# rl-tools/raptor

Measured on AMD Instinct MI355X. Metric: env-steps/sec (whole node) at 65536 quadrotors per GPU, higher is better.
Workload: dtype f32; 1 GPU; 65536 parallel quadrotors per GPU, fp32 RK4 dynamics + fp32 GRU actor (RAPTOR checkpoint), domain-randomised params, auto-reset, fused rollout; envs_per_gpu=65536, total_envs=65536, episode_length=500, parallelism=single GPU, mode=fused, engine=hip, device=AMD Radeon Graphics, exchange=none (one rank: nothing to gather)

## Files before the change

### include/raptor_quad.h

```cpp
#ifndef RAPTOR_QUAD_H
#define RAPTOR_QUAD_H

#include <stddef.h>
#include <stdint.h>

#ifdef __cplusplus
extern "C" {
#endif

#define RQ_ABI_VERSION 5

#if defined(__GNUC__)
#define RQ_API __attribute__((visibility("default")))
#else
#define RQ_API
#endif

#define RQ_POLICY_INPUT_DIM 22
#define RQ_POLICY_HIDDEN_DIM 16
#define RQ_POLICY_OUTPUT_DIM 4
#define RQ_POLICY_NUM_WEIGHTS 2084
#define RQ_ACTION_DIM 4
#define RQ_OBSERVATION_DIM 26

// ... 378 lines not shown
RQ_API int rq_allgather_returns(rq_env* env, rq_comm* comm);
RQ_API int rq_comm_gathered(rq_comm* comm, const float** dev_ptr, uint32_t* count, float* host_out);

RQ_API int rq_device_timer_start(rq_device* dev);
RQ_API int rq_device_timer_stop(rq_device* dev, float* elapsed_ms);
RQ_API int rq_device_set_rollout_timing(rq_device* dev, int enable);
RQ_API int rq_device_last_rollout_ms(rq_device* dev, float* kernel_ms);
RQ_API int rq_device_last_rollout_waves(rq_device* dev, uint64_t* records, uint32_t capacity, uint32_t* n_waves);
RQ_API int rq_device_last_rollout_clock(rq_device* dev, float* core_ghz);
RQ_API int rq_device_launch_floor(rq_device* dev, uint32_t n, uint32_t reps, float* us_per_launch);
RQ_API int rq_device_set_speculation(rq_device* dev, int enable);
RQ_API int rq_device_set_resident(rq_device* dev, int enable);
RQ_API int rq_device_get_resident(const rq_device* dev, int* enabled, int* running, uint64_t* starts, uint64_t* commands, uint64_t* replays);
RQ_API int rq_device_get_resident_timing(const rq_device* dev, uint64_t* ticks6);
RQ_API int rq_device_get_speculation(const rq_device* dev, int* enabled, int* suspended, uint32_t* consecutive_misses);

#ifdef __cplusplus
}
#endif
#endif
```

### raptor_amd/_lib.py

```python
import ctypes as C
import os

_PKG = os.path.dirname(os.path.abspath(__file__))
LIB_PATH = os.environ.get("RAPTOR_QUAD_LIB") or os.path.join(_PKG, "libraptor_quad.so")

POLICY_INPUT_DIM = 22
POLICY_HIDDEN_DIM = 16
POLICY_OUTPUT_DIM = 4
POLICY_NUM_WEIGHTS = 2084
ACTION_DIM = 4
OBSERVATION_DIM = 26
PARAM_DIM = 26
STATE_DIM = 27

ROLLOUT_FUSED, ROLLOUT_CHAINED = 0, 1
ROLLOUT_AUTORESET = 1
POLICY_FP32, POLICY_BF16_MFMA, POLICY_F16X2_MFMA = 0, 1, 2
ACT_IDENTITY, ACT_RELU, ACT_TANH = 0, 1, 2
COMM_ID_BYTES = 128


class RaptorQuadError(RuntimeError):
    def __init__(self, status, message):
        super().__init__(f"libraptor_quad status {status}: {message}")
# ... 51 lines not shown
    "rq_last_error": [],
    "rq_status_string": [C.c_int],
    "rq_device_count": [C.POINTER(C.c_int)],
    "rq_device_create": [C.c_int, C.POINTER(_vp)],
    "rq_device_destroy": [_vp],
    "rq_device_synchronize": [_vp],
    "rq_device_timer_start": [_vp],
    "rq_device_timer_stop": [_vp, _fp],
    "rq_device_launch_floor": [_vp, C.c_uint32, C.c_uint32, _fp],
    "rq_device_set_rollout_timing": [_vp, C.c_int],
    "rq_device_last_rollout_ms": [_vp, _fp],
    "rq_device_last_rollout_waves": [_vp, C.c_void_p, C.c_uint32, _u32p],
    "rq_device_last_rollout_clock": [_vp, _fp],
    "rq_device_set_speculation": [_vp, C.c_int],
    "rq_device_get_speculation": [_vp, C.POINTER(C.c_int), C.POINTER(C.c_int), _u32p],
    "rq_device_set_resident": [_vp, C.c_int],
    "rq_device_get_resident_timing": [_vp, C.POINTER(C.c_uint64)],
    "rq_device_get_resident": [_vp, C.POINTER(C.c_int), C.POINTER(C.c_int), C.POINTER(C.c_uint64), C.POINTER(C.c_uint64), C.POINTER(C.c_uint64)],
    "rq_device_stream": [_vp, C.POINTER(_vp)],
    "rq_rng_create": [_vp, C.POINTER(_vp)],
    "rq_rng_destroy": [_vp],
    "rq_initialize_rng": [_vp, _vp, C.c_uint64],
    "rq_rng_get": [_vp, C.POINTER(C.c_uint64), _u32p],
    "rq_rng_set_epoch": [_vp, C.c_uint32],
    "rq_env_create": [_vp, C.c_uint32, C.c_uint64, C.POINTER(_vp)],
    "rq_env_destroy": [_vp],
    "rq_env_num_envs": [_vp, _u32p],
    "rq_env_leading_dim": [_vp, _u32p],
    "rq_env_default_config": [C.POINTER(EnvConfig)],
    "rq_initialize_environment": [_vp, _vp],
# ... 292 lines not shown
```

### raptor_amd/csrc/rq_capi.cpp

```cpp
#include "rq_objects.hpp"

namespace rq {

thread_local std::string g_last_error;
thread_local int tl_scope_depth = 0, tl_scope_device = -1;

int fail(int status, const std::string& msg) {
    try { g_last_error = msg; } catch (...) { g_last_error.clear(); }
    return status;
}

}

namespace rqh {

bool device_registry(const void* dev, int op) {
    static std::mutex m;
    static std::unordered_set<const void*> live;
    std::lock_guard<std::mutex> lock(m);
    if (op > 0) { live.insert(dev); return true; }
    if (op < 0) { live.erase(dev); return false; }
    return live.count(dev) != 0;
}

// ... 167 lines not shown
    DeviceScope on_device(ordinal);
    if (on_device.rc) return on_device.rc;
    rq_device* d = new (std::nothrow) rq_device();
    RQ_REQUIRE(d, RQ_ERR_OUT_OF_MEMORY, "host allocation failed");
    d->ordinal = ordinal;
    hipError_t e1 = hipStreamCreateWithFlags(&d->stream, hipStreamNonBlocking);
    hipError_t e2 = hipEventCreate(&d->ev_start);
    hipError_t e3 = hipEventCreate(&d->ev_stop);
    if (e3 == hipSuccess) e3 = hipEventCreateWithFlags(&d->ev_h2d, hipEventDisableTiming);
    if (e1 != hipSuccess || e2 != hipSuccess || e3 != hipSuccess) {
        delete d;
        return fail(RQ_ERR_HIP, "rq_device_create: stream/event creation failed");
    }
    d->graphs_enabled = std::getenv("RQ_NO_GRAPHS") == nullptr;
    small_batch_setup(d);
    resident_setup(d);
    device_registry(d, +1);
    *out = d;
    return RQ_OK;
}

RQ_API int rq_device_destroy(rq_device* dev) {
    if (!dev) return RQ_OK;
    DeviceScope on_device(dev->ordinal);
    resident_teardown(dev);
    device_registry(dev, -1);
    if (dev->stream) { (void)hipStreamSynchronize(dev->stream); (void)hipStreamDestroy(dev->stream); }
    if (dev->ev_start) (void)hipEventDestroy(dev->ev_start);
    if (dev->ev_stop) (void)hipEventDestroy(dev->ev_stop);
    if (dev->ev_h2d) (void)hipEventDestroy(dev->ev_h2d);
// ... 106 lines not shown
    DeviceScope on_device(dev); int rc = on_device.rc; if (rc) return rc;
    RQ_HIP(dev->rows.reserve(dev->stream, n));
    for (int i = 0; i < 3; ++i) RQ_HIP(rq::launch_fill_f32(dev->stream, dev->rows, 0.0f, n));
    RQ_HIP(hipEventRecord(dev->ev_start, dev->stream));
    for (uint32_t i = 0; i < reps; ++i) RQ_HIP(rq::launch_fill_f32(dev->stream, dev->rows, 0.0f, n));
    RQ_HIP(hipEventRecord(dev->ev_stop, dev->stream));
    RQ_HIP(hipEventSynchronize(dev->ev_stop));
    float ms = 0.0f;
    RQ_HIP(hipEventElapsedTime(&ms, dev->ev_start, dev->ev_stop));
    *us_per_launch = ms * 1e3f / (float)reps;
    return RQ_OK;
}

RQ_API int rq_device_stream(rq_device* dev, void** hip_stream) {
    RQ_REQUIRE(dev && hip_stream, RQ_ERR_INVALID_ARGUMENT, "null argument");
    *hip_stream = (void*)dev->stream;
    return RQ_OK;
}

RQ_API int rq_rng_create(rq_device* dev, rq_rng** out) {
    RQ_REQUIRE(dev && out, RQ_ERR_INVALID_ARGUMENT, "null argument");
    rq_rng* r = new (std::nothrow) rq_rng();
    RQ_REQUIRE(r, RQ_ERR_OUT_OF_MEMORY, "host allocation failed");
    r->dev = dev;
    *out = r;
    return RQ_OK;
}

RQ_API int rq_rng_destroy(rq_rng* rng) { delete rng; return RQ_OK; }

// ... 148 lines not shown
    delete p;
    return RQ_OK;
}
RQ_API int rq_params_get(const rq_params* p, float* host_out) {
    RQ_REQUIRE(p && host_out, RQ_ERR_INVALID_ARGUMENT, "null argument");
    return soa_to_host(p->env->dev, p->d, p->env->n, p->env->ld, RQ_PARAM_DIM, host_out);
}
RQ_API int rq_params_set(rq_params* p, const float* host_in) {
    RQ_REQUIRE(p && host_in, RQ_ERR_INVALID_ARGUMENT, "null argument");
    p->version = fresh_version();
    return host_to_soa(p->env->dev, host_in, p->env->n, RQ_PARAM_DIM, p->env->ld, RQ_PARAM_DIM, p->d);
}
RQ_API int rq_params_device_ptr(const rq_params* p, float** dev_ptr) {
    RQ_REQUIRE(p && dev_ptr, RQ_ERR_INVALID_ARGUMENT, "null argument");
    const_cast<rq_params*>(p)->exposed = true;
    *dev_ptr = p->d; return RQ_OK;
}

RQ_API int rq_state_create(rq_env* env, rq_state** out) {
    RQ_REQUIRE(env && out, RQ_ERR_INVALID_ARGUMENT, "null argument");
    DeviceScope on_device(env->dev); int rc = on_device.rc; if (rc) return rc;
    rq_state* s = new (std::nothrow) rq_state();
    RQ_REQUIRE(s, RQ_ERR_OUT_OF_MEMORY, "host allocation failed");
    s->env = env; s->ordinal = env->ordinal;
    const size_t bytes = (size_t)RQ_STATE_DIM * env->ld * sizeof(float);
    hipError_t e = hipMalloc(&s->d, bytes);
    s->refs = new (std::nothrow) int(1);
    if (e != hipSuccess || !s->refs) {
        if (e == hipSuccess) (void)hipFree(s->d);
        delete s->refs; delete s;
// ... 86 lines not shown
```

### raptor_amd/csrc/rq_capi_rollout.cpp

```cpp
#include "rq_objects.hpp"

#include <cmath>

namespace rqh {

int traj_block_to_host(rq_device* dev, const float* d_soa, uint32_t steps, uint32_t n, uint32_t ld, uint32_t dim,
                              float* host) {
    const size_t per_step = (size_t)n * dim * sizeof(float);
    uint32_t chunk = (uint32_t)std::min<size_t>(steps, std::max<size_t>(1, ((size_t)1 << 30) / per_step));
    if (chunk > 65535u) chunk = 65535u;
    RQ_HIP(dev->rows.reserve(dev->stream, (size_t)n * dim * chunk));
    for (uint32_t s0 = 0; s0 < steps; s0 += chunk) {
        const uint32_t c = std::min(chunk, steps - s0);
        RQ_HIP(rq::launch_soa_to_rows(dev->stream, d_soa + (size_t)s0 * dim * ld, ld, dim, n, dev->rows, c));
        RQ_HIP(hipMemcpyAsync(host + (size_t)s0 * n * dim, dev->rows, per_step * c, hipMemcpyDeviceToHost, dev->stream));
        RQ_HIP(hipStreamSynchronize(dev->stream));
    }
    return RQ_OK;
}

int rollout_check(RolloutFrame& f, const RolloutCall& c, bool actor) {
    const rq_trajectory* traj = c.traj;
    int rc = check_env_objects(c.dev, c.env, c.params, c.state); if (rc) return rc;
    RQ_REFUSE(c.who, c.params && c.state && actor && c.rng, RQ_ERR_INVALID_ARGUMENT, "null argument");
// ... 119 lines not shown
    rq_device* dev = c.dev;
    if (dev->k_timing && c.n_steps) {
        const uint32_t waves = (c.env->n + 63u) / 64u;
        const hipError_t e = dev->k_span.reserve(dev->stream, (size_t)waves * 5);
        if (e != hipSuccess) return hip_failed(c.who, "dev->k_span.reserve(dev->stream, (size_t)waves * 5)", e);
        dev->k_span_used = waves;
    }
    a.span = dev->k_timing ? dev->k_span.get() : nullptr;
    const hipError_t e = rq::launch_rollout_fused(dev->stream, a);
    if (e != hipSuccess) return hip_failed(c.who, "rq::launch_rollout_fused", e);
    dev->k_timed = dev->k_timing && c.n_steps > 0;
    dev->k_fetched = false;
    return RQ_OK;
}

}

using namespace rqh;

namespace {

struct PolicyActor {
    static constexpr bool kFoldAndReplay = true;
    rq_policy* policy;
    bool given() const { return policy != nullptr; }
    int check(const RolloutCall& c, const RolloutFrame& f) const {
        RQ_REFUSE(c.who, policy->dev == c.dev, RQ_ERR_SHAPE_MISMATCH, "policy lives on another device");
        RQ_REFUSE(c.who, !c.tables || policy->sas_mode == RQ_SAS_OFF, RQ_ERR_INVALID_ARGUMENT,
                  "tracked rollouts do not carry the SampleAndSquash stage");
        for (int k = 0; k < kScheduleKinds && c.mode == RQ_ROLLOUT_FUSED; ++k) {
            if (!f.sched[k].rows) continue;
            if (policy->precision != RQ_POLICY_FP32) return refuses_fused(c.who, k, "a bf16 / f16x2 policy");
            if (policy->sas_mode != RQ_SAS_OFF) return refuses_fused(c.who, k, "a policy with a SampleAndSquash stage");
        }
        return RQ_OK;
    }
    int prepare(const RolloutCall& c) const {
        const int rc = policy_size(policy, c.env->n); if (rc) return rc;
        RQ_REFUSE(c.who, policy->ld == c.env->ld, RQ_ERR_SHAPE_MISMATCH, "policy batch does not match the env");
        return RQ_OK;
    }
    int fused(const RolloutCall& c, const RolloutFrame& f) const {
        rq::FusedArgs a = fused_args(c, f);
        a.hidden = policy->hidden; a.weights = policy->w_dev;
        a.precision = policy->precision; a.images = packed_of(policy); a.interval = policy->native_interval;
        a.sas = sas_of(policy, c.rng->epoch, nullptr, c.env->offset);
        return fused_launch(c, a);
    }
    rq::EnvStepLaunch env_step(const RolloutCall& c, const RolloutFrame& f) const {
        rq::EnvStepLaunch e = env_step_launch(c, f);
        e.hidden = policy->hidden; e.weights = policy->w_dev;
        return e;
    }
    hipError_t thaw(const RolloutCall& c, const RolloutFrame& f) const { return rq::launch_thaw_frozen(c.dev->stream, env_step(c, f)); }
    hipError_t act(const RolloutCall& c, const RolloutFrame&, uint32_t epoch, const uint32_t* epoch_base) const {
        const rq_env* env = c.env;
        rq::ActorStepLaunch a;
        a.n = env->n; a.packed = packed_of(policy); a.precision = policy->precision;
        a.obs = env->obs; a.ld_obs = env->ld; a.hidden = policy->hidden; a.ld_h = policy->ld; a.act = env->act; a.ld_act = env->ld;
        a.frozen = env->st.frozen;
        a.sas = sas_of(policy, epoch, epoch_base, env->offset);
// ... 94 lines not shown
}

template <typename T>
int env_schedule_get(const char* who, int kind, const rq_env* env, T** bank, uint32_t* id_out) {
    RQ_REFUSE(who, env && bank, RQ_ERR_INVALID_ARGUMENT, "null argument");
    const auto& slot = env->schedule[kind];
    *bank = static_cast<T*>(slot.bank);
    if (slot.bank && id_out) std::memcpy(id_out, slot.ids.data(), (size_t)env->n * sizeof(uint32_t));
    return RQ_OK;
}

}

extern "C" {

RQ_API int rq_rollout(rq_device* dev, rq_env* env, const rq_params* params, rq_state* state, rq_policy* policy,
               rq_rng* rng, uint32_t n_steps, int mode, uint32_t flags) {
    return rollout_run({__func__, dev, env, params, state, rng, n_steps, mode, flags, nullptr, nullptr, nullptr}, PolicyActor{policy});
}

RQ_API int rq_rollout_record(rq_device* dev, rq_env* env, const rq_params* params, rq_state* state, rq_policy* policy,
                      rq_rng* rng, uint32_t n_steps, int mode, uint32_t flags, rq_trajectory* trajectory) {
    RQ_REQUIRE(trajectory, RQ_ERR_INVALID_ARGUMENT, "null trajectory");
    return rollout_run({__func__, dev, env, params, state, rng, n_steps, mode, flags, trajectory, nullptr, nullptr}, PolicyActor{policy});
}

RQ_API int rq_rollout_track(rq_device* dev, rq_env* env, const rq_params* params, rq_state* state, rq_policy* policy,
                     rq_rng* rng, uint32_t n_steps, int mode, uint32_t flags, rq_trajectory* trajectory,
                     const rq_reference* reference) {
    RQ_REQUIRE(reference, RQ_ERR_INVALID_ARGUMENT, "null reference");
// ... 164 lines not shown
```

### raptor_amd/csrc/rq_host.hpp

```cpp
#pragma once
#include <hip/hip_runtime_api.h>

#include <cstdint>
#include <string>

#include "../../include/raptor_quad.h"

namespace rq {

int fail(int status, const std::string& msg);

extern thread_local int tl_scope_depth, tl_scope_device;

struct DeviceScope {
    int previous = -1, target, rc = RQ_OK;
    bool nested = false;
    explicit DeviceScope(int ordinal) : target(ordinal) {
        if (tl_scope_depth > 0 && tl_scope_device == target) { nested = true; ++tl_scope_depth; return; }
        if (hipGetDevice(&previous) != hipSuccess) previous = -1;
        if (previous != target) {
            const hipError_t e = hipSetDevice(target);
            if (e != hipSuccess) rc = fail(RQ_ERR_HIP, std::string("hipSetDevice -> ") + hipGetErrorString(e));
        }
        outer_depth = tl_scope_depth; outer_device = tl_scope_device;
        tl_scope_depth = 1; tl_scope_device = target;
    }
    explicit DeviceScope(const rq_device* dev);
    DeviceScope(const rq_device* dev, struct KeepResident);
    ~DeviceScope() {
        if (nested) { --tl_scope_depth; return; }
        tl_scope_depth = outer_depth; tl_scope_device = outer_device;
        if (previous >= 0 && previous != target) (void)hipSetDevice(previous);
    }
// ... 34 lines not shown
```

### raptor_amd/csrc/rq_kernels.hpp

```cpp
#pragma once
#include <hip/hip_runtime_api.h>
#include <stdint.h>
#include "../../include/raptor_quad.h"
#include "rq_fused_route.hpp"
#include "rq_loss_launch.hpp"
#include "rq_step_launch.hpp"

namespace rq {

inline StepCfg step_cfg(const rq_env_config& c) {
    return {c.dt, c.gravity, c.episode_step_limit, c.reward_scale, c.reward_constant,
            c.reward_termination_penalty, c.reward_position, c.reward_orientation,
            c.reward_linear_velocity, c.reward_angular_velocity, c.reward_action,
            c.termination_enabled, c.termination_position, c.termination_linear_velocity,
            c.termination_angular_velocity, c.action_history_raw};
}
inline NoiseCfg noise_cfg(const rq_env_config& c) {
    return {c.noise_position, c.noise_orientation, c.noise_linear_velocity, c.noise_angular_velocity};
}
inline bool noise_enabled(const rq_env_config& c) {
    return c.noise_position > 0.f || c.noise_orientation > 0.f || c.noise_linear_velocity > 0.f ||
           c.noise_angular_velocity > 0.f;
}
inline SampleCfg sample_cfg(const rq_env_config& c) {
// ... 5 lines not shown
}

struct TrajPtrs {
    float* obs; float* act; float* rew; uint8_t* done;
    uint32_t t0;
};

struct TrackPtrs {
    const float* ref;
    uint32_t rows;
    uint32_t row0_at;
    float* sq;
    uint32_t* steps;
};
static_assert(sizeof(TrackPtrs) == 32, "the kernels' argument blocks hold TrackPtrs by value");

struct ResidentArgs {
    Batch b; StepCfg c; SampleCfg sc; uint64_t seed;
    const float* params; float* act; StatsPtrs st;
    float* obs_buf[2];
    const float* packed;
    float* hidden[2];
    uint32_t ld_h; float* pol_act;
    const float* rows_action;
    const uint32_t* small_rows;
    float* rows_obs;
    float* rows_act;
    uint32_t* flag;
    volatile uint32_t* packet;
    uint32_t* exited;
// ... 153 lines not shown
    bool noise = false, autoreset = false;
    const float* params = nullptr; float* state = nullptr; float* hidden = nullptr;
    const float* weights = nullptr;
    StatsPtrs st{};
    TrajPtrs traj{};
    TrackPtrs trk{};
    WrenchPtrs wr{};
    VehiclePtrs vh{};
    WindPtrs wd{};
    int precision = RQ_POLICY_FP32;
    const float* images = nullptr; const uint32_t* block_policy = nullptr; const uint32_t* policy_interval = nullptr;
    SasArgs sas{};
    uint32_t interval = 1;
    bool bank_rated = false;
    unsigned long long* span = nullptr;
};
inline FusedTraits fused_traits(const FusedArgs& a) {
    return {a.b.n, a.precision, a.sas.mode != RQ_SAS_OFF, a.trk.ref != nullptr, a.wr.rows != nullptr, a.interval,
            a.block_policy != nullptr, a.bank_rated, a.vh.rows != nullptr, a.wd.rows != nullptr};
}
hipError_t launch_rollout_fused(hipStream_t s, const FusedArgs& a);
hipError_t launch_soa_to_rows(hipStream_t s, const float* soa, uint32_t ld, uint32_t dim, uint32_t n, float* rows,
                              uint32_t slabs = 1);
hipError_t launch_rows_to_soa(hipStream_t s, const float* rows, uint32_t stride, uint32_t dim, uint32_t n, uint32_t ld,
                              float* soa);

hipError_t launch_fill_f32(hipStream_t s, float* p, float v, uint32_t count);

}
```

### raptor_amd/csrc/rq_objects.hpp

```cpp
#pragma once
#include <hip/hip_runtime_api.h>

#include <algorithm>
#include <atomic>
#include <cstdint>
#include <cstdio>
#include <cstdlib>
#include <cstring>
#include <ctime>
#include <emmintrin.h>
#include <mutex>
#include <new>
#include <string>
#include <unordered_set>
#include <utility>
#include <vector>

#include "../../include/raptor_quad.h"
#include "rq_kernels.hpp"

#include "rq_host.hpp"
#include "rq_memory.hpp"
#include "rq_call_memory.hpp"
#include "rq_env_schedule.hpp"
// ... 68 lines not shown
    const rq_params* params = nullptr; uint64_t params_version = 0;
    const rq_state* state[2] = {nullptr, nullptr};
    uint64_t version[2] = {0, 0};
    uint32_t seq = 0, n = 0;
    bool in_alt = false;
};
struct Speculation {
    bool enabled = true;
    rq_policy* last_policy = nullptr;
    rq_policy* policy = nullptr; uint64_t policy_version = 0;
    uint32_t batch = 0, seq = 0, oc_seq = 0;
    bool outstanding = false;
    bool suspended = false; uint32_t misses = 0;
};
constexpr uint32_t kSpeculationMissLimit = 4;

struct rq_device {
    int ordinal = 0;
    hipStream_t stream = nullptr;
    hipEvent_t ev_start = nullptr, ev_stop = nullptr;
    DeviceBuffer<unsigned long long> k_span;
    uint32_t k_span_used = 0;
    std::vector<unsigned long long> k_host;
    bool k_fetched = false;
    double k_ticks_per_ms = 1e5;
    bool graphs_enabled = true;
    uint32_t graph_fallbacks = 0;
    bool k_timing = false;
    bool k_timed = false;
    PinnedBuffer<float> staging;
    DeviceBuffer<float> rows;
    DeviceBuffer<float> rows2;
    PinnedBuffer<float> staging_in;
    hipEvent_t ev_h2d = nullptr;
    bool h2d_pending = false;
    HostMailbox mailbox;
    ObservationCache obs_cache;
    Speculation spec;
    ResidentExecutor resident;
};
struct rq_rng {
    rq_device* dev = nullptr;
    uint64_t seed = 0;
    uint32_t epoch = 0;
    uint32_t param_epoch = 0;
    bool initialized = false;
};

namespace rqh {
struct RowTables {
    const rq_device* dev = nullptr;
    int ordinal = 0;
    uint32_t n_tables = 0, rows = 0;
// ... 292 lines not shown
int require_bank_native_rate(const rq_policy_bank* bank, const char* what);

struct RolloutCall {
    const char* who;
    rq_device* dev; rq_env* env; const rq_params* params; rq_state* state; rq_rng* rng;
    uint32_t n_steps; int mode; uint32_t flags; rq_trajectory* traj;
    const RowTables* tables;
    const uint32_t* reference_id;
};
struct RolloutFrame {
    rq::TrajPtrs tp{nullptr, nullptr, nullptr, nullptr, 0};
    rq::TrackPtrs trk{};
    uint64_t row0_gen = 0;
    SchedulePtrs sched[kScheduleKinds];
    rq::Batch b; rq::StepCfg sc; rq::NoiseCfg nc; rq::SampleCfg smp; bool noise;
};
#define RQ_REFUSE(who, cond, status, msg)                                          \
    do {                                                                           \
        if (!(cond)) return rq::fail((status), std::string(who) + ": " + (msg));   \
    } while (0)
int rollout_check(RolloutFrame& f, const RolloutCall& c, bool actor);
int rollout_check_tables(const RolloutCall& c);
int rollout_track(RolloutFrame& f, const RolloutCall& c);
int rollout_begin(RolloutFrame& f, const RolloutCall& c);
void rollout_end(const RolloutCall& c);
int first_rows_failed(const char* what, const rq::FirstRowsStatus& s);
inline int hip_failed(const char* who, const char* what, hipError_t e) {
    return fail(e == hipErrorOutOfMemory ? RQ_ERR_OUT_OF_MEMORY : RQ_ERR_HIP, std::string(who) + ": " + what + " -> " + hipGetErrorString(e));
}
#define RQ_HIP_AS(who, expr)                                                \
    do {                                                                    \
        const hipError_t e_ = (expr);                                       \
        if (e_ != hipSuccess) return rqh::hip_failed((who), #expr, e_);     \
    } while (0)
rq::FusedArgs fused_args(const RolloutCall& c, const RolloutFrame& f);
int fused_launch(const RolloutCall& c, rq::FusedArgs& a);
rq::EnvStepLaunch env_step_launch(const RolloutCall& c, const RolloutFrame& f);

constexpr uint32_t kGraphSteps = 25;
constexpr size_t kMaxGraphs = 8;

template <typename Actor>
int rollout_chained(const RolloutCall& c, const RolloutFrame& f, const Actor& actor) {
    rq_device* dev = c.dev; rq_env* env = c.env; const rq_rng* rng = c.rng;
    const uint32_t n_steps = c.n_steps;
    const bool fold = Actor::kFoldAndReplay && !c.traj;
    const char* what = "";
    auto one_step = [&](uint32_t epoch, const uint32_t* epoch_base, uint32_t t_record) -> hipError_t {
        hipError_t e = hipSuccess;
        if (!fold) {
            what = "rq::launch_observe";
// ... 61 lines not shown
                    RQ_HIP(hipGraphLaunch(exec, dev->stream));
            }
        }
    }
    for (uint32_t t = done_steps; t < n_steps; ++t)
        if ((e = one_step(rng->epoch + t, nullptr, t)) != hipSuccess) return hip_failed(c.who, what, e);
    return RQ_OK;
}

template <typename Actor>
int rollout_run(const RolloutCall& c, Actor actor) {
    RolloutFrame f;
    int rc = rollout_check(f, c, actor.given()); if (rc) return rc;
    rc = actor.check(c, f); if (rc) return rc;
    rc = rollout_check_tables(c); if (rc) return rc;
    DeviceScope on_device(c.dev); rc = on_device.rc; if (rc) return rc;
    rc = actor.prepare(c); if (rc) return rc;
    rc = rollout_track(f, c); if (rc) return rc;
    rc = rollout_begin(f, c); if (rc) return rc;
    rc = c.mode == RQ_ROLLOUT_FUSED ? actor.fused(c, f) : rollout_chained(c, f, actor); if (rc) return rc;
    rollout_end(c);
    return RQ_OK;
}
int traj_block_to_host(rq_device* dev, const float* d_soa, uint32_t steps, uint32_t n, uint32_t ld, uint32_t dim, float* host);

template <typename T>
int copy_out(const rq_env* env, const T* src, T* dst, int dst_is_device) {
    RQ_REQUIRE(env && dst, RQ_ERR_INVALID_ARGUMENT, "null argument");
    DeviceScope on_device(env->dev); int rc = on_device.rc; if (rc) return rc;
    RQ_REQUIRE(CallMemory::valid(dst_is_device), RQ_ERR_INVALID_ARGUMENT, "dst_is_device must be 0, 1 or 2");
    CallMemory mem(dst_is_device, env->dev->stream, env->dev->ordinal);
    RQ_HIP(hipMemcpyAsync(dst, src, (size_t)env->n * sizeof(T),
                          dst_is_device ? hipMemcpyDeviceToDevice : hipMemcpyDeviceToHost, env->dev->stream));
    RQ_HIP(mem.finish());
    return RQ_OK;
}
// ... 14 lines not shown
```

### raptor_amd/csrc/rq_rollout.hpp

```cpp
#pragma once
#include <hip/hip_ext.h>

#include <cstdlib>
#include <type_traits>

#include "rq_device_math.hpp"
#include "rq_dispatch.hpp"

namespace rq {

static constexpr int kBlock = 256;
static constexpr int kFusedBlock = 64;

template <bool NT, class T>
__device__ __forceinline__ void put(T* p, T v) {
    if constexpr (NT) __builtin_nontemporal_store(v, p);
    else *p = v;
}
static constexpr bool kNtObs = true, kNtTraj = true;
static constexpr int kNtTrajAux = 2;

__device__ __forceinline__ uint32_t env_index() { return blockIdx.x * blockDim.x + threadIdx.x; }

template <typename T>
__device__ __forceinline__ T* field(T* base, uint32_t f, uint32_t ld) { return base + (size_t)f * ld; }

template <typename A> struct WavesPerSimd { static constexpr int value = 1; static constexpr bool bf16 = false; };
template <> struct WavesPerSimd<ActorF32Lean> { static constexpr int value = 2; static constexpr bool bf16 = false; };
template <> struct WavesPerSimd<ActorBF16> { static constexpr int value = 1; static constexpr bool bf16 = true; };
template <> struct WavesPerSimd<ActorF16X2> { static constexpr int value = 1; static constexpr bool bf16 = true; };


template <bool NOISE, bool AUTORESET, bool RECORD, bool SAS, typename ACTOR>
__global__ __launch_bounds__(kFusedBlock, WavesPerSimd<ACTOR>::value) void k_rollout_fused(Batch b, StepCfg c, NoiseCfg nc, SampleCfg sc,
                                                               uint64_t seed, uint32_t epoch0, uint32_t n_steps,
                                                               const float* __restrict__ params,
                                                               float* __restrict__ state,
                                                               float* __restrict__ hidden,
                                                               const float* __restrict__ w,
                                                               const float* __restrict__ packed, StatsPtrs st,
                                                               TrajPtrs traj, SasArgs sas,
                                                               unsigned long long* __restrict__ span) {
    constexpr bool TRACK = false, RATE = false, WRENCH = false;
    constexpr TrackPtrs trk{};
    constexpr WrenchPtrs wr{};
    constexpr bool VEHICLE = false;
    constexpr VehiclePtrs vh{};
    constexpr bool WIND = false;
    constexpr WindPtrs wd{};
    constexpr uint32_t interval = 1;
#include "rq_rollout_body.inc"
}

template <bool NOISE, bool AUTORESET, bool RECORD, typename ACTOR>
__global__ __launch_bounds__(kFusedBlock, WavesPerSimd<ACTOR>::value) void k_rollout_fused_track(Batch b, StepCfg c, NoiseCfg nc, SampleCfg sc,
                                                               uint64_t seed, uint32_t epoch0, uint32_t n_steps,
                                                               const float* __restrict__ params,
                                                               float* __restrict__ state,
                                                               float* __restrict__ hidden,
                                                               const float* __restrict__ w,
                                                               const float* __restrict__ packed, StatsPtrs st,
                                                               TrajPtrs traj, TrackPtrs trk,
                                                               unsigned long long* __restrict__ span) {
    constexpr bool TRACK = true, SAS = false, RATE = false, WRENCH = false;
    constexpr SasArgs sas{};
    constexpr WrenchPtrs wr{};
// ... 21 lines not shown
    constexpr bool VEHICLE = false;
    constexpr VehiclePtrs vh{};
    constexpr bool WIND = false;
    constexpr WindPtrs wd{};
#include "rq_rollout_body.inc"
}

hipError_t launch_rollout_fused_16bit(hipStream_t s, const FusedArgs& a, FusedFamily family);

inline unsigned fused_grid(const FusedArgs& a) { return (a.b.n + kFusedBlock - 1) / kFusedBlock; }

template <bool SAS, typename ACTOR>
inline void launch_fused_actor(hipStream_t s, const FusedArgs& a) {
    dispatch_bools([&](auto NZ, auto AR, auto RC) {
        hipLaunchKernelGGL((k_rollout_fused<NZ(), AR(), RC(), SAS, ACTOR>), dim3(fused_grid(a)), dim3(kFusedBlock), 0, s,
                           a.b, a.c, a.nc, a.sc, a.seed, a.epoch0, a.n_steps, a.params, a.state, a.hidden, a.weights, a.images,
                           a.st, a.traj, a.sas, a.span);
    }, a.noise, a.autoreset, a.traj.obs != nullptr);
}

template <typename ACTOR>
inline void launch_fused_track_actor(hipStream_t s, const FusedArgs& a) {
    dispatch_bools([&](auto NZ, auto AR, auto RC) {
        hipLaunchKernelGGL((k_rollout_fused_track<NZ(), AR(), RC(), ACTOR>), dim3(fused_grid(a)), dim3(kFusedBlock), 0, s,
                           a.b, a.c, a.nc, a.sc, a.seed, a.epoch0, a.n_steps, a.params, a.state, a.hidden, a.weights, a.images,
                           a.st, a.traj, a.trk, a.span);
    }, a.noise, a.autoreset, a.traj.obs != nullptr);
}

template <typename ACTOR>
inline void launch_fused_rate_actor(hipStream_t s, const FusedArgs& a) {
// ... 9 lines not shown
```

### raptor_amd/csrc/rq_rollout_body.inc

```
    unsigned long long t_in = 0;
    if (span != nullptr) t_in = (unsigned long long)wall_clock64();
    const uint32_t i0 = env_index();
    const uint32_t wave_base = i0 & ~63u;
    const uint32_t i = i0 < b.n ? i0 : b.n - 1;
    const bool valid = i0 < b.n;
    const size_t ld = b.ld;
    const uint64_t genv = b.env_offset + i;
    uint32_t ep = AUTORESET ? st.episode[i] : 0u;
    float hover_rpm = 0.0f;
    if (AUTORESET) hover_rpm = field(params, RQ_P_HOVER_RPM, ld)[i];
    const EnvConsts k = make_consts([&](int f) { return field(params, f, ld)[i]; });
    QuadState y;
    f32x2 LA01, LA23;
    float f6[6], hQ[4][4];
    y.load([&](int j) { return field(state, j, ld)[i]; });
    LA01 = f32x2{field(state, (RQ_S_LAST_ACTION + 0), ld)[i], field(state, (RQ_S_LAST_ACTION + 1), ld)[i]};
    LA23 = f32x2{field(state, (RQ_S_LAST_ACTION + 2), ld)[i], field(state, (RQ_S_LAST_ACTION + 3), ld)[i]};
#pragma unroll
    for (int j = 0; j < 6; ++j) f6[j] = field(state, (RQ_S_FORCE + j), ld)[i];
    load_hidden_q(hidden, ld, wave_base, b.n, hQ);
    float ep_ret = st.returns[i];
    uint32_t ep_steps = st.steps[i];
    float last_r = st.last_reward[i];
    float trk_sq = 0.0f;
// ... 259 lines not shown
                    if ((ended_mask & ~pre_mask) != 0) refill();
                }
                if (ended) {
                    take_presampled();
                    ds = make_disturbance(k, c.gravity, f6);
                }
                pre_mask &= ~ended_mask;
                select_hidden_q(ended_mask, h0Q, hQ);
                actor.reset_carry(ended_mask, hQ, carry);
            }
        }
    }
    };
    unsigned long long t_loop = 0, t_done = 0, c_loop = 0, c_done = 0;
    if (span != nullptr) { t_loop = (unsigned long long)wall_clock64(); c_loop = (unsigned long long)__builtin_readcyclecounter(); }
    if (sym_tau) rollout_loop(std::true_type{});
    else         rollout_loop(std::false_type{});
    if (span != nullptr) { c_done = (unsigned long long)__builtin_readcyclecounter(); t_done = (unsigned long long)wall_clock64(); }

    const bool commit = AUTORESET || !was_frozen;
    if (!AUTORESET && n_steps > 0 && last_step + 1 != n_steps) last_d = 4;
    if (AUTORESET) last_d = last_t ? 1 : (ep_steps == 0 ? 2 : 0);
    uint32_t ie = i;
    asm volatile("" : "+v"(ie));
    size_t lde = ld;
    asm volatile("" : "+s"(lde));
    if (valid && commit) {
        y.store([&](int j, float v) { field(state, j, lde)[ie] = v; });
        field(state, (RQ_S_LAST_ACTION + 0), lde)[ie] = LA01[0]; field(state, (RQ_S_LAST_ACTION + 1), lde)[ie] = LA01[1];
        field(state, (RQ_S_LAST_ACTION + 2), lde)[ie] = LA23[0]; field(state, (RQ_S_LAST_ACTION + 3), lde)[ie] = LA23[1];
        st.returns[ie] = ep_ret;
        st.steps[ie] = ep_steps;
// ... 25 lines not shown
```

### raptor_amd/l2f.py

```python
import ctypes as C
import json
import weakref

import numpy as np

from . import _lib, schedules
from ._lib import (ACTION_DIM, OBSERVATION_DIM, PARAM_DIM, STATE_DIM, ROLLOUT_AUTORESET, ROLLOUT_CHAINED,
                   ROLLOUT_FUSED, EnvConfig, RaptorQuadError)

__all__ = ["Device", "Reference", "WrenchBank", "VehicleBank", "WindBank", "UI", "vector", "vector8", "EnvConfig", "RaptorQuadError"]


class UI:

    def __init__(self, ns=""):
        self.ns = ns


class Device:

    def __init__(self, ordinal=0):
        h = C.c_void_p()
        _lib.call("rq_device_create", int(ordinal), C.byref(h))
        self._h = h
# ... 33 lines not shown
        _lib.call("rq_device_last_rollout_clock", self._h, C.byref(ghz))
        return float(ghz.value)

    def launch_floor(self, n, reps=200):
        us = C.c_float()
        _lib.call("rq_device_launch_floor", self._h, int(n), int(reps), C.byref(us))
        return float(us.value)

    def set_speculation(self, enable):
        _lib.call("rq_device_set_speculation", self._h, 1 if enable else 0)

    def speculation(self):
        e, s, m = C.c_int(), C.c_int(), C.c_uint32()
        _lib.call("rq_device_get_speculation", self._h, C.byref(e), C.byref(s), C.byref(m))
        return {"enabled": bool(e.value), "suspended": bool(s.value), "consecutive_misses": int(m.value)}

    def set_resident(self, enable):
        _lib.call("rq_device_set_resident", self._h, 1 if enable else 0)

    def resident(self):
        e, r = C.c_int(), C.c_int()
        a, b, c = C.c_uint64(), C.c_uint64(), C.c_uint64()
        _lib.call("rq_device_get_resident", self._h, C.byref(e), C.byref(r), C.byref(a), C.byref(b), C.byref(c))
        return {"enabled": bool(e.value), "running": bool(r.value), "starts": int(a.value), "commands": int(b.value), "replays": int(c.value)}

    def resident_timing_us(self):
        t = (C.c_uint64 * 6)()
        _lib.call("rq_device_get_resident_timing", self._h, t)
        return {k: (int(t[i + 1]) - int(t[0])) / 100.0 for i, k in enumerate(("rows_read", "stepped", "first_flag", "acted", "done"))}

# ... 696 lines not shown
```

Baseline: 22.96 billion env-steps/s.

## Let a running fused rollout kernel absorb steps from later rollout calls

```diff
diff --git a/include/raptor_quad.h b/include/raptor_quad.h
--- a/include/raptor_quad.h
+++ b/include/raptor_quad.h
@@ -416,6 +416,8 @@
 RQ_API int rq_device_get_resident(const rq_device* dev, int* enabled, int* running, uint64_t* starts, uint64_t* commands, uint64_t* replays);
 RQ_API int rq_device_get_resident_timing(const rq_device* dev, uint64_t* ticks6);
 RQ_API int rq_device_get_speculation(const rq_device* dev, int* enabled, int* suspended, uint32_t* consecutive_misses);
+RQ_API int rq_device_set_rollout_extension(rq_device* dev, int enable);
+RQ_API int rq_device_get_rollout_extension(rq_device* dev, int* enabled, uint64_t* launches, uint64_t* absorbed, uint64_t* continued);
 
 #ifdef __cplusplus
 }
diff --git a/raptor_amd/_lib.py b/raptor_amd/_lib.py
--- a/raptor_amd/_lib.py
+++ b/raptor_amd/_lib.py
@@ -89,6 +89,8 @@
     "rq_device_last_rollout_clock": [_vp, _fp],
     "rq_device_set_speculation": [_vp, C.c_int],
     "rq_device_get_speculation": [_vp, C.POINTER(C.c_int), C.POINTER(C.c_int), _u32p],
+    "rq_device_set_rollout_extension": [_vp, C.c_int],
+    "rq_device_get_rollout_extension": [_vp, C.POINTER(C.c_int), C.POINTER(C.c_uint64), C.POINTER(C.c_uint64), C.POINTER(C.c_uint64)],
     "rq_device_set_resident": [_vp, C.c_int],
     "rq_device_get_resident_timing": [_vp, C.POINTER(C.c_uint64)],
     "rq_device_get_resident": [_vp, C.POINTER(C.c_int), C.POINTER(C.c_int), C.POINTER(C.c_uint64), C.POINTER(C.c_uint64), C.POINTER(C.c_uint64)],
diff --git a/raptor_amd/csrc/rq_capi.cpp b/raptor_amd/csrc/rq_capi.cpp
--- a/raptor_amd/csrc/rq_capi.cpp
+++ b/raptor_amd/csrc/rq_capi.cpp
@@ -4,6 +4,7 @@
 
 thread_local std::string g_last_error;
 thread_local int tl_scope_depth = 0, tl_scope_device = -1;
+std::atomic<uint64_t> g_scopes_entered[kScopeCounters];
 
 int fail(int status, const std::string& msg) {
     try { g_last_error = msg; } catch (...) { g_last_error.clear(); }
@@ -205,6 +206,7 @@
     }
     d->graphs_enabled = std::getenv("RQ_NO_GRAPHS") == nullptr;
     small_batch_setup(d);
+    d->extend.enabled = std::getenv("RQ_NO_ROLLOUT_EXTENSION") == nullptr;
     resident_setup(d);
     device_registry(d, +1);
     *out = d;
@@ -341,6 +343,7 @@
 
 RQ_API int rq_device_stream(rq_device* dev, void** hip_stream) {
     RQ_REQUIRE(dev && hip_stream, RQ_ERR_INVALID_ARGUMENT, "null argument");
+    rq::scope_entered(dev->ordinal);
     *hip_stream = (void*)dev->stream;
     return RQ_OK;
 }
@@ -519,6 +522,7 @@
 RQ_API int rq_params_device_ptr(const rq_params* p, float** dev_ptr) {
     RQ_REQUIRE(p && dev_ptr, RQ_ERR_INVALID_ARGUMENT, "null argument");
     const_cast<rq_params*>(p)->exposed = true;
+    rq::scope_entered(p->ordinal);
     *dev_ptr = p->d; return RQ_OK;
 }
 
diff --git a/raptor_amd/csrc/rq_capi_rollout.cpp b/raptor_amd/csrc/rq_capi_rollout.cpp
--- a/raptor_amd/csrc/rq_capi_rollout.cpp
+++ b/raptor_amd/csrc/rq_capi_rollout.cpp
@@ -157,6 +157,54 @@
     return RQ_OK;
 }
 
+int extend_plan(const RolloutCall& c, const RolloutFrame& f, const rq_policy* pol, uint64_t version_in, bool ready_in, rq::FusedArgs& a) {
+    rq_device* dev = c.dev;
+    RolloutExtension& x = dev->extend;
+    const bool was_open = x.open;
+    x.open = false; x.pending = false;
+    if (!x.enabled || dev->k_timing || !rq::fused_extends(a) || c.params->exposed || c.state->exposed || c.n_steps >= rq::kExtendMaxTotal)
+        return RQ_OK;
+    if (x.agree.empty()) {
+        RQ_HIP_AS(c.who, x.agree.alloc(2));
+        RQ_HIP_AS(c.who, hipMemsetAsync(x.agree, 0, 2 * sizeof(unsigned long long), dev->stream));
+    }
+    if (x.request.empty()) {
+        RQ_HIP_AS(c.who, x.request.alloc(1));
+        *x.request.get() = 0;
+    }
+    const bool continues = was_open && ready_in && x.scopes == f.scopes_in && x.env == c.env && x.env_uid == c.env->uid &&
+                           std::memcmp(&x.cfg, &c.env->cfg, sizeof(rq_env_config)) == 0 && x.params == c.params &&
+                           x.params_version == c.params->version && x.params_d == a.params && x.state == c.state &&
+                           x.state_version == c.state->version && x.state_d == a.state && x.policy == pol &&
+                           x.policy_version == version_in && x.weight_version == pol->weight_version && x.hidden == a.hidden &&
+                           x.image == a.images && x.rng == c.rng && x.seed == a.seed && x.next_epoch == a.epoch0 &&
+                           x.total + c.n_steps <= rq::kExtendMaxTotal;
+    x.seq = (x.seq + 1) & 0x7FFFFFFFu;
+    if (x.seq == 0) x.seq = 1;
+    if (continues) { a.ext.start = x.total; x.total += c.n_steps; ++x.continued; }
+    else           { a.ext.start = 0; x.total = c.n_steps; ++x.window; }
+    __atomic_store_n(x.request.get(), ((unsigned long long)x.window << 32) | x.total, __ATOMIC_RELEASE);
+    a.ext.agree = x.agree; a.ext.request = x.request; a.ext.counts = reinterpret_cast<uint32_t*>(x.agree.get() + 1);
+    a.ext.seq = x.seq; a.ext.window = x.window; a.ext.epoch0 = a.epoch0;
+    x.env = c.env; x.env_uid = c.env->uid; x.cfg = c.env->cfg;
+    x.params = c.params; x.params_version = c.params->version; x.params_d = a.params;
+    x.state = c.state; x.state_d = a.state;
+    x.policy = pol; x.policy_version = pol->version; x.weight_version = pol->weight_version; x.hidden = a.hidden; x.image = a.images;
+    x.rng = c.rng; x.seed = a.seed;
+    x.pending = true;
+    return RQ_OK;
+}
+
+void extend_launched(const RolloutCall& c) {
+    RolloutExtension& x = c.dev->extend;
+    if (!x.pending) return;
+    x.pending = false;
+    x.open = true;
+    x.state_version = c.state->version; x.next_epoch = c.rng->epoch;
+    x.scopes = rq::scopes_entered(c.dev->ordinal);
+    ++x.launches;
+}
+
 }
 
 using namespace rqh;
@@ -167,8 +215,11 @@
     static constexpr bool kFoldAndReplay = true;
     rq_policy* policy;
     bool given() const { return policy != nullptr; }
+    mutable uint64_t version_in = 0;
+    mutable bool ready_in = false;
     int check(const RolloutCall& c, const RolloutFrame& f) const {
         RQ_REFUSE(c.who, policy->dev == c.dev, RQ_ERR_SHAPE_MISMATCH, "policy lives on another device");
+        version_in = policy->version; ready_in = !policy->needs_reset && policy->batch == c.env->n && !policy->hidden.empty();
         RQ_REFUSE(c.who, !c.tables || policy->sas_mode == RQ_SAS_OFF, RQ_ERR_INVALID_ARGUMENT,
                   "tracked rollouts do not carry the SampleAndSquash stage");
         for (int k = 0; k < kScheduleKinds && c.mode == RQ_ROLLOUT_FUSED; ++k) {
@@ -188,6 +239,7 @@
         a.hidden = policy->hidden; a.weights = policy->w_dev;
         a.precision = policy->precision; a.images = packed_of(policy); a.interval = policy->native_interval;
         a.sas = sas_of(policy, c.rng->epoch, nullptr, c.env->offset);
+        const int rc = extend_plan(c, f, policy, version_in, ready_in, a); if (rc) return rc;
         return fused_launch(c, a);
     }
     rq::EnvStepLaunch env_step(const RolloutCall& c, const RolloutFrame& f) const {
@@ -312,6 +364,28 @@
 
 extern "C" {
 
+RQ_API int rq_device_set_rollout_extension(rq_device* dev, int enable) {
+    RQ_REQUIRE(dev, RQ_ERR_INVALID_ARGUMENT, "null argument");
+    dev->extend.enabled = enable != 0;
+    dev->extend.open = false;
+    return RQ_OK;
+}
+
+RQ_API int rq_device_get_rollout_extension(rq_device* dev, int* enabled, uint64_t* launches, uint64_t* absorbed, uint64_t* continued) {
+    RQ_REQUIRE(dev, RQ_ERR_INVALID_ARGUMENT, "null argument");
+    DeviceScope on_device(dev); int rc = on_device.rc; if (rc) return rc;
+    uint32_t counts[2] = {0, 0};
+    if (!dev->extend.agree.empty()) {
+        RQ_HIP(hipMemcpyAsync(counts, dev->extend.agree.get() + 1, sizeof(counts), hipMemcpyDeviceToHost, dev->stream));
+        RQ_HIP(hipStreamSynchronize(dev->stream));
+    }
+    if (enabled) *enabled = dev->extend.enabled ? 1 : 0;
+    if (launches) *launches = dev->extend.launches;
+    if (absorbed) *absorbed = counts[0];
+    if (continued) *continued = counts[1];
+    return RQ_OK;
+}
+
 RQ_API int rq_rollout(rq_device* dev, rq_env* env, const rq_params* params, rq_state* state, rq_policy* policy,
                rq_rng* rng, uint32_t n_steps, int mode, uint32_t flags) {
     return rollout_run({__func__, dev, env, params, state, rng, n_steps, mode, flags, nullptr, nullptr, nullptr}, PolicyActor{policy});
diff --git a/raptor_amd/csrc/rq_host.hpp b/raptor_amd/csrc/rq_host.hpp
--- a/raptor_amd/csrc/rq_host.hpp
+++ b/raptor_amd/csrc/rq_host.hpp
@@ -1,6 +1,7 @@
 #pragma once
 #include <hip/hip_runtime_api.h>
 
+#include <atomic>
 #include <cstdint>
 #include <string>
 
@@ -12,11 +13,17 @@
 
 extern thread_local int tl_scope_depth, tl_scope_device;
 
+constexpr int kScopeCounters = 64;
+extern std::atomic<uint64_t> g_scopes_entered[kScopeCounters];
+inline uint64_t scopes_entered(int ordinal) { return g_scopes_entered[(unsigned)ordinal % kScopeCounters].load(std::memory_order_relaxed); }
+inline void scope_entered(int ordinal) { g_scopes_entered[(unsigned)ordinal % kScopeCounters].fetch_add(1, std::memory_order_relaxed); }
+
 struct DeviceScope {
     int previous = -1, target, rc = RQ_OK;
     bool nested = false;
     explicit DeviceScope(int ordinal) : target(ordinal) {
         if (tl_scope_depth > 0 && tl_scope_device == target) { nested = true; ++tl_scope_depth; return; }
+        scope_entered(target);
         if (hipGetDevice(&previous) != hipSuccess) previous = -1;
         if (previous != target) {
             const hipError_t e = hipSetDevice(target);
diff --git a/raptor_amd/csrc/rq_kernels.hpp b/raptor_amd/csrc/rq_kernels.hpp
--- a/raptor_amd/csrc/rq_kernels.hpp
+++ b/raptor_amd/csrc/rq_kernels.hpp
@@ -43,6 +43,18 @@
     uint32_t* steps;
 };
 static_assert(sizeof(TrackPtrs) == 32, "the kernels' argument blocks hold TrackPtrs by value");
+
+struct ExtendPtrs {
+    unsigned long long* agree = nullptr;
+    const unsigned long long* request = nullptr;
+    uint32_t* counts = nullptr;
+    uint32_t seq = 0;
+    uint32_t window = 0;
+    uint32_t start = 0;
+    uint32_t epoch0 = 0;
+};
+constexpr unsigned long long kExtendClosed = 1ull << 63;
+constexpr uint32_t kExtendMaxTotal = 1u << 30;
 
 struct ResidentArgs {
     Batch b; StepCfg c; SampleCfg sc; uint64_t seed;
@@ -226,10 +238,16 @@
     uint32_t interval = 1;
     bool bank_rated = false;
     unsigned long long* span = nullptr;
+    ExtendPtrs ext{};
 };
 inline FusedTraits fused_traits(const FusedArgs& a) {
     return {a.b.n, a.precision, a.sas.mode != RQ_SAS_OFF, a.trk.ref != nullptr, a.wr.rows != nullptr, a.interval,
             a.block_policy != nullptr, a.bank_rated, a.vh.rows != nullptr, a.wd.rows != nullptr};
+}
+inline bool fused_extends(const FusedArgs& a) {
+    const FusedRoute r = route_fused(fused_traits(a));
+    return r.family == FusedFamily::PLAIN && r.build == FusedBuild::F32 && !r.vehicle && !r.wind && a.autoreset &&
+           a.traj.obs == nullptr && a.span == nullptr && a.b.n > 0 && a.n_steps > 0;
 }
 hipError_t launch_rollout_fused(hipStream_t s, const FusedArgs& a);
 hipError_t launch_soa_to_rows(hipStream_t s, const float* soa, uint32_t ld, uint32_t dim, uint32_t n, float* rows,
diff --git a/raptor_amd/csrc/rq_objects.hpp b/raptor_amd/csrc/rq_objects.hpp
--- a/raptor_amd/csrc/rq_objects.hpp
+++ b/raptor_amd/csrc/rq_objects.hpp
@@ -106,6 +106,22 @@
     bool suspended = false; uint32_t misses = 0;
 };
 constexpr uint32_t kSpeculationMissLimit = 4;
+struct RolloutExtension {
+    bool enabled = true;
+    DeviceBuffer<unsigned long long> agree;
+    PinnedBuffer<unsigned long long> request;
+    uint32_t seq = 0, window = 0;
+    bool open = false;
+    bool pending = false;
+    uint32_t total = 0;
+    uint64_t scopes = 0;
+    const rq_env* env = nullptr; uint64_t env_uid = 0; rq_env_config cfg{};
+    const rq_params* params = nullptr; uint64_t params_version = 0; const float* params_d = nullptr;
+    const rq_state* state = nullptr; uint64_t state_version = 0; const float* state_d = nullptr;
+    const rq_policy* policy = nullptr; uint64_t policy_version = 0, weight_version = 0; const float* hidden = nullptr; const float* image = nullptr;
+    const rq_rng* rng = nullptr; uint64_t seed = 0; uint32_t next_epoch = 0;
+    uint64_t launches = 0, continued = 0;
+};
 
 struct rq_device {
     int ordinal = 0;
@@ -129,6 +145,7 @@
     HostMailbox mailbox;
     ObservationCache obs_cache;
     Speculation spec;
+    RolloutExtension extend;
     ResidentExecutor resident;
 };
 struct rq_rng {
@@ -451,6 +468,7 @@
     uint64_t row0_gen = 0;
     SchedulePtrs sched[kScheduleKinds];
     rq::Batch b; rq::StepCfg sc; rq::NoiseCfg nc; rq::SampleCfg smp; bool noise;
+    uint64_t scopes_in = 0;
 };
 #define RQ_REFUSE(who, cond, status, msg)                                          \
     do {                                                                           \
@@ -472,6 +490,8 @@
     } while (0)
 rq::FusedArgs fused_args(const RolloutCall& c, const RolloutFrame& f);
 int fused_launch(const RolloutCall& c, rq::FusedArgs& a);
+int extend_plan(const RolloutCall& c, const RolloutFrame& f, const rq_policy* pol, uint64_t version_in, bool ready_in, rq::FusedArgs& a);
+void extend_launched(const RolloutCall& c);
 rq::EnvStepLaunch env_step_launch(const RolloutCall& c, const RolloutFrame& f);
 
 constexpr uint32_t kGraphSteps = 25;
@@ -563,12 +583,14 @@
     int rc = rollout_check(f, c, actor.given()); if (rc) return rc;
     rc = actor.check(c, f); if (rc) return rc;
     rc = rollout_check_tables(c); if (rc) return rc;
+    f.scopes_in = rq::scopes_entered(c.dev->ordinal);
     DeviceScope on_device(c.dev); rc = on_device.rc; if (rc) return rc;
     rc = actor.prepare(c); if (rc) return rc;
     rc = rollout_track(f, c); if (rc) return rc;
     rc = rollout_begin(f, c); if (rc) return rc;
     rc = c.mode == RQ_ROLLOUT_FUSED ? actor.fused(c, f) : rollout_chained(c, f, actor); if (rc) return rc;
     rollout_end(c);
+    extend_launched(c);
     return RQ_OK;
 }
 int traj_block_to_host(rq_device* dev, const float* d_soa, uint32_t steps, uint32_t n, uint32_t ld, uint32_t dim, float* host);
diff --git a/raptor_amd/csrc/rq_rollout.hpp b/raptor_amd/csrc/rq_rollout.hpp
--- a/raptor_amd/csrc/rq_rollout.hpp
+++ b/raptor_amd/csrc/rq_rollout.hpp
@@ -30,9 +30,39 @@
 template <> struct WavesPerSimd<ActorBF16> { static constexpr int value = 1; static constexpr bool bf16 = true; };
 template <> struct WavesPerSimd<ActorF16X2> { static constexpr int value = 1; static constexpr bool bf16 = true; };
 
+__device__ __forceinline__ unsigned long long extend_uniform(unsigned long long v) {
+    const uint32_t lo = __builtin_amdgcn_readfirstlane((uint32_t)v), hi = __builtin_amdgcn_readfirstlane((uint32_t)(v >> 32));
+    return ((unsigned long long)hi << 32) | lo;
+}
+__device__ __forceinline__ unsigned long long extend_agreed(const unsigned long long* agree) {
+    return extend_uniform(__hip_atomic_load(agree, __ATOMIC_ACQUIRE, __HIP_MEMORY_SCOPE_AGENT));
+}
+__device__ __forceinline__ unsigned long long extend_requested(const unsigned long long* request) {
+    return extend_uniform(__hip_atomic_load(request, __ATOMIC_ACQUIRE, __HIP_MEMORY_SCOPE_SYSTEM));
+}
+__device__ __forceinline__ bool extend_propose(unsigned long long* agree, unsigned long long seen, unsigned long long want) {
+    bool won = false;
+    if (__builtin_amdgcn_mbcnt_hi(~0u, __builtin_amdgcn_mbcnt_lo(~0u, 0u)) == 0)
+        won = __hip_atomic_compare_exchange_strong(agree, &seen, want, __ATOMIC_ACQ_REL, __ATOMIC_ACQUIRE, __HIP_MEMORY_SCOPE_AGENT);
+    return won;
+}
+__device__ __forceinline__ ExtendPtrs extend_args_again() {
+#if __HIP_DEVICE_COMPILE__
+    const __attribute__((address_space(4))) ExtendPtrs* p =
+        (const __attribute__((address_space(4))) ExtendPtrs*)__builtin_amdgcn_kernarg_segment_ptr();
+    asm volatile("" : "+s"(p));
+    return *p;
+#else
+    return ExtendPtrs{};
+#endif
+}
+__device__ __forceinline__ uint32_t extend_total(unsigned long long w) { return (uint32_t)w; }
+__device__ __forceinline__ uint32_t extend_owner(unsigned long long w) { return (uint32_t)(w >> 32) & 0x7FFFFFFFu; }
+__device__ __forceinline__ unsigned long long extend_word(uint32_t seq, uint32_t total) { return ((unsigned long long)seq << 32) | total; }
+
 
 template <bool NOISE, bool AUTORESET, bool RECORD, bool SAS, typename ACTOR>
-__global__ __launch_bounds__(kFusedBlock, WavesPerSimd<ACTOR>::value) void k_rollout_fused(Batch b, StepCfg c, NoiseCfg nc, SampleCfg sc,
+__global__ __launch_bounds__(kFusedBlock, WavesPerSimd<ACTOR>::value) void k_rollout_fused(ExtendPtrs ext, Batch b, StepCfg c, NoiseCfg nc, SampleCfg sc,
                                                                uint64_t seed, uint32_t epoch0, uint32_t n_steps,
                                                                const float* __restrict__ params,
                                                                float* __restrict__ state,
@@ -49,7 +79,10 @@
     constexpr bool WIND = false;
     constexpr WindPtrs wd{};
     constexpr uint32_t interval = 1;
+    constexpr bool kExtend = AUTORESET && !RECORD && !SAS && WavesPerSimd<ACTOR>::value == 1 && !WavesPerSimd<ACTOR>::bf16;
+#define RQ_BODY_EXTEND 1
 #include "rq_rollout_body.inc"
+#undef RQ_BODY_EXTEND
 }
 
 template <bool NOISE, bool AUTORESET, bool RECORD, typename ACTOR>
@@ -101,7 +134,7 @@
 inline void launch_fused_actor(hipStream_t s, const FusedArgs& a) {
     dispatch_bools([&](auto NZ, auto AR, auto RC) {
         hipLaunchKernelGGL((k_rollout_fused<NZ(), AR(), RC(), SAS, ACTOR>), dim3(fused_grid(a)), dim3(kFusedBlock), 0, s,
-                           a.b, a.c, a.nc, a.sc, a.seed, a.epoch0, a.n_steps, a.params, a.state, a.hidden, a.weights, a.images,
+                           a.ext, a.b, a.c, a.nc, a.sc, a.seed, a.epoch0, a.n_steps, a.params, a.state, a.hidden, a.weights, a.images,
                            a.st, a.traj, a.sas, a.span);
     }, a.noise, a.autoreset, a.traj.obs != nullptr);
 }
diff --git a/raptor_amd/csrc/rq_rollout_body.inc b/raptor_amd/csrc/rq_rollout_body.inc
--- a/raptor_amd/csrc/rq_rollout_body.inc
+++ b/raptor_amd/csrc/rq_rollout_body.inc
@@ -1,5 +1,22 @@
     unsigned long long t_in = 0;
     if (span != nullptr) t_in = (unsigned long long)wall_clock64();
+#ifdef RQ_BODY_EXTEND
+    if constexpr (kExtend) {
+        if (ext.agree != nullptr) {
+            const uint32_t ext_reached = ext.start + n_steps;
+            const unsigned long long seen = extend_agreed(ext.agree);
+            if (extend_owner(seen) != ext.seq) {
+                if (ext.start != 0 && extend_total(seen) >= ext_reached) {
+                    if (blockIdx.x == 0 && threadIdx.x == 0)
+                        (void)__hip_atomic_fetch_add(&ext.counts[0], 1u, __ATOMIC_RELAXED, __HIP_MEMORY_SCOPE_AGENT);
+                    return;
+                }
+                if (extend_propose(ext.agree, seen, extend_word(ext.seq, ext_reached)) && ext.start != 0)
+                    (void)__hip_atomic_fetch_add(&ext.counts[1], 1u, __ATOMIC_RELAXED, __HIP_MEMORY_SCOPE_AGENT);
+            }
+        }
+    }
+#endif
     const uint32_t i0 = env_index();
     const uint32_t wave_base = i0 & ~63u;
     const uint32_t i = i0 < b.n ? i0 : b.n - 1;
@@ -297,8 +314,29 @@
     };
     unsigned long long t_loop = 0, t_done = 0, c_loop = 0, c_done = 0;
     if (span != nullptr) { t_loop = (unsigned long long)wall_clock64(); c_loop = (unsigned long long)__builtin_readcyclecounter(); }
+#ifdef RQ_BODY_EXTEND
+    for (;;) {
+        if (sym_tau) rollout_loop(std::true_type{});
+        else         rollout_loop(std::false_type{});
+        if constexpr (!kExtend) break;
+        const ExtendPtrs ex = extend_args_again();
+        if (ex.agree == nullptr) break;
+        uint32_t ext_reached = ex.start + (epoch0 - ex.epoch0) + n_steps;
+        unsigned long long agreed = extend_agreed(ex.agree);
+        if (agreed == extend_word(ex.seq, ext_reached)) {
+            const unsigned long long asked = extend_requested(ex.request);
+            const bool more = (uint32_t)(asked >> 32) == ex.window && (uint32_t)asked > ext_reached && (uint32_t)asked <= kExtendMaxTotal;
+            (void)extend_propose(ex.agree, agreed, more ? extend_word(ex.seq, (uint32_t)asked) : agreed | kExtendClosed);
+            agreed = extend_agreed(ex.agree);
+        }
+        if (extend_owner(agreed) != ex.seq || extend_total(agreed) <= ext_reached) break;
+        epoch0 += n_steps;
+        n_steps = extend_total(agreed) - ext_reached;
+    }
+#else
     if (sym_tau) rollout_loop(std::true_type{});
     else         rollout_loop(std::false_type{});
+#endif
     if (span != nullptr) { c_done = (unsigned long long)__builtin_readcyclecounter(); t_done = (unsigned long long)wall_clock64(); }
 
     const bool commit = AUTORESET || !was_frozen;
diff --git a/raptor_amd/l2f.py b/raptor_amd/l2f.py
--- a/raptor_amd/l2f.py
+++ b/raptor_amd/l2f.py
@@ -71,6 +71,15 @@
         e, s, m = C.c_int(), C.c_int(), C.c_uint32()
         _lib.call("rq_device_get_speculation", self._h, C.byref(e), C.byref(s), C.byref(m))
         return {"enabled": bool(e.value), "suspended": bool(s.value), "consecutive_misses": int(m.value)}
+
+    def set_rollout_extension(self, enable):
+        _lib.call("rq_device_set_rollout_extension", self._h, 1 if enable else 0)
+
+    def rollout_extension(self):
+        e = C.c_int()
+        a, b, c = C.c_uint64(), C.c_uint64(), C.c_uint64()
+        _lib.call("rq_device_get_rollout_extension", self._h, C.byref(e), C.byref(a), C.byref(b), C.byref(c))
+        return {"enabled": bool(e.value), "launches": int(a.value), "absorbed": int(b.value), "continued": int(c.value)}
 
     def set_resident(self, enable):
         _lib.call("rq_device_set_resident", self._h, 1 if enable else 0)
```

Result: slower. 22.64 billion env-steps/s (-1.4%).
